# Sindhu-Hegde/jegal

Hardware: AMD Instinct MI355X
Metric: clips/sec (T=150 frames, 270x480) embedding extraction (higher is better)
Workload: dtype f16; 1 GPU; BASELINE configs[1]: synthetic batch=32 gesture-only (GestSync conv + JEGAL gesture encoder), uint8 150x270x480x3 clips resident in HBM, seeded synthetic weights; clips_per_gpu=32, frames=150, precision_mode=5, chunk=32, conv1_zero_tile_skip=True, dual_stream=True, parallelism=clip-sharded x1, no data-path collective

## Files before the change

### jegal_amd/csrc/conv1.hip

```cpp
#include "common.h"

#ifdef JG_CLOCK_STAMPS
__device__ unsigned long long jg_clock_stamps_conv1[2 * 1024];
extern "C" int jg_clock_read_conv1(unsigned long long* out, int n) {
    return hipMemcpyFromSymbol(out, HIP_SYMBOL(jg_clock_stamps_conv1), sizeof(unsigned long long) * (n < 2048 ? n : 2048)) == hipSuccess ? 0 : 1;
}
#endif
#include <cstdio>
#include <cstdlib>
#include <cstring>

struct Conv1Args {
    const uint8_t* src;
    int nclip, T, pad, P;
    const f16* Wd;
    float scale;
    f16* out;
    f16* edge;
    f16* dump;
    int nstrips;
    float invP;
    int zskip;
    const unsigned* zmask;
    const f16* zconst;
    int fill_partial;
};

namespace {
constexpr int IH = 270, IW = 480;
constexpr int PH = 43, PW = 78;
constexpr int TROWS = 16;
constexpr int ROW_PITCH = 3744;
constexpr int TILE_BYTES = TROWS * ROW_PITCH;
__device__ __host__ constexpr int slot_off(int x) { return 32 * x + 16 * (x / 3); }
constexpr int ROW_TILES = 22, COL_TILES = 5;
constexpr int CONV_BYTES = 4 * 8 * 32 * 16;
constexpr int CARRY_BYTES = 8 * 32 * 16;
constexpr int OFF_CONV = 2 * TILE_BYTES;
constexpr int OFF_CARRY = OFF_CONV + 2 * CONV_BYTES;
constexpr int OFF_INIT = OFF_CARRY + 2 * CARRY_BYTES;
constexpr int OFF_LIVE = OFF_INIT + 32;
constexpr int OFF_SKIP = OFF_INIT + 256;
constexpr int MAX_WG_STRIPS = 640;
constexpr int LDS_BYTES = OFF_SKIP + 4 * MAX_WG_STRIPS;
constexpr int MAX_WGS = 1024;
constexpr int DUMP_HALVES_PER_WG = 256 * 8;
}

typedef uint32_t u32x3 __attribute__((ext_vector_type(3)));
struct C1Regs { u32x3 w[2][5]; };

__device__ __forceinline__ f16x8 max8(f16x8 a, f16x8 b) {
    return __builtin_elementwise_max(a, b);
}

__device__ __forceinline__ int conv1_s2_of_mask(unsigned sk) {
    const int L = __builtin_ctz(~sk);
    constexpr int C2_OH = (PH - 5) / 2 + 1;
    const int rs = L >= 2 ? L - 2 : 0;
    return rs < C2_OH ? rs : C2_OH - 1;
}

struct Strips {
    int s_lo, r_hi, GX;
    const unsigned* tab;
    bool use_skip;
    __device__ __forceinline__ bool any() const { return s_lo < r_hi && GX > 0; }
    __device__ __forceinline__ unsigned zero_bands(int k) const {
        return use_skip ? (unsigned)__builtin_amdgcn_readfirstlane((int)tab[k]) : 0u;
    }
};
__device__ __forceinline__ Strips conv1_strips(const Conv1Args& a, const char* smem) {
    const int G32 = (int)gridDim.x;
    const int xcd = blockIdx.x & 7, xidx = blockIdx.x >> 3;
    const int GX = (G32 + 7 - xcd) >> 3;
    const int per = (a.nstrips + 7) >> 3;
    const int r_lo = xcd * per, r_hi = (r_lo + per < a.nstrips) ? r_lo + per : a.nstrips;
    return Strips{r_lo + xidx, r_hi, GX, reinterpret_cast<const unsigned*>(smem + OFF_SKIP), a.zmask != nullptr};
}
__device__ __forceinline__ void strip_split(int strip, int& nf, int& j) {
    nf = (int)((unsigned)strip / 5u);
    j = strip - nf * 5;
}
__device__ __forceinline__ unsigned skip_of(unsigned z) { return z & ((z << 1) | 1u); }
struct Walk {
    int strip, rt;
    int k;
    unsigned skip;
    unsigned z;
    bool done;
};
template <class F>
__device__ __forceinline__ void walk_next(const Strips& S, Walk& q, F&& on_strip) {
    if (q.done) return;
    while (true) {
        if (++q.rt == ROW_TILES) {
            q.rt = 0;
            q.strip += S.GX;
            ++q.k;
            if (q.strip >= S.r_hi) { q.done = true; return; }
            q.z = S.zero_bands(q.k);
            q.skip = skip_of(q.z);
            on_strip(q.strip, q.skip);
        }
        if (!((q.skip >> q.rt) & 1u)) return;
    }
}
template <class F>
__device__ __forceinline__ Walk walk_first(const Strips& S, F&& on_strip) {
    Walk q = {S.s_lo, -1, 0, 0u, 0u, !S.any()};
    if (q.done) return q;
    q.z = S.zero_bands(0);
    q.skip = skip_of(q.z);
    on_strip(q.strip, q.skip);
    walk_next(S, q, on_strip);
    return q;
}

__device__ __forceinline__ bool tile_live(const char* smem, int t) {
    return __builtin_amdgcn_readfirstlane(*reinterpret_cast<const int*>(smem + OFF_LIVE + (t & 1) * 4)) != 0;
}
__device__ __forceinline__ bool tile_is_zero(const char* smem, int t) {
    const int4 fl = *reinterpret_cast<const int4*>(smem + OFF_INIT + (t & 1) * 16);
    return __builtin_amdgcn_readfirstlane(fl.x | fl.y | fl.z | fl.w) == 0;
}

struct Mfma32 {
    static constexpr int NSTEP = 49, NCB = 1;
    static constexpr int DEPTH = 6;
    typedef f32x16 Acc;
    const int chalf, r, h;
    f16x8 wreg[49];
    const char* base;
    __device__ __forceinline__ Mfma32(const f16* Wd, int lane, int chalf_) : chalf(chalf_), r(lane & 31), h(lane >> 5) {
#pragma unroll
        for (int s = 0; s < 49; ++s)
            wreg[s] = *reinterpret_cast<const f16x8*>(Wd + conv1_wd_index(s, chalf * 32 + r, 8 * h));
    }
    __device__ __forceinline__ void set_tile(const char* cur) { base = cur + 112 * r + 16 * h; }
    __device__ __forceinline__ f16x8 frag(int gi) const {
        const int q = gi / 49, s = gi - q * 49;
        const int kh = s / 7, kw = s - kh * 7;
        return *reinterpret_cast<const f16x8*>(base + (6 * q + kh) * ROW_PITCH + 32 * kw + 16 * (kw / 3));
    }
    __device__ __forceinline__ static void zero(Acc& acc) {
#pragma unroll
        for (int x = 0; x < 16; ++x) acc[x] = 0.f;
    }
    __device__ __forceinline__ void step(Acc& acc, int s, int, f16x8 f) const {
        acc = __builtin_amdgcn_mfma_f32_32x32x16_f16(wreg[s], f, acc, 0, 0, 0);
    }
    __device__ __forceinline__ void store(const Acc& acc, char* cbuf, int mb, float scale) const {
#pragma unroll
        for (int g = 0; g < 4; ++g) {
            const f16x4 hv = {(f16)fmaxf(acc[4 * g] * scale, 0.f), (f16)fmaxf(acc[4 * g + 1] * scale, 0.f),
                              (f16)fmaxf(acc[4 * g + 2] * scale, 0.f), (f16)fmaxf(acc[4 * g + 3] * scale, 0.f)};
            *reinterpret_cast<f16x4*>(cbuf + ((mb * 8 + chalf * 4 + g) * 32 + r) * 16 + 8 * h) = hv;
        }
    }
};
struct Mfma16 {
    static constexpr int NSTEP = 25, NCB = 2;
    static constexpr int DEPTH = 4;
    struct Acc { f32x4 v[2][2]; };
    const int chalf, n16, kq, sel, half, colp;
    f16x8 wreg[25][2];
    int lb_row, lb_32, lb_224;
    int st_off;
    const char *p_row, *p_32, *p_224;
    __device__ __forceinline__ static void step_slots(int t, int& kha, int& kwa, int& khb, int& kwb) {
        if (t < 21) { kha = 2 * (t / 7); kwa = t % 7; khb = kha + 1; kwb = kwa; }
        else if (t == 21) { kha = khb = 6; kwa = 1; kwb = 2; }
        else if (t == 22) { kha = khb = 6; kwa = 4; kwb = 5; }
        else if (t == 23) { kha = khb = 6; kwa = 0; kwb = 6; }
        else { kha = khb = 6; kwa = 3; kwb = 4; }
    }
    __device__ __forceinline__ Mfma16(const f16* Wd, int lane, int chalf_)
        : chalf(chalf_), n16(lane & 15), kq(lane >> 4), sel(kq & 1), half(kq >> 1),
          colp((n16 >= 4 && n16 < 12) ? 2 * (n16 - 4) : (n16 < 4 ? 2 * n16 + 1 : 2 * (n16 - 8) + 1)) {
#pragma unroll
        for (int t = 0; t < 25; ++t) {
            int kha, kwa, khb, kwb;
            step_slots(t, kha, kwa, khb, kwb);
            const int sl = sel ? khb * 7 + kwb : kha * 7 + kwa;
#pragma unroll
            for (int ob = 0; ob < 2; ++ob) {
                wreg[t][ob] = *reinterpret_cast<const f16x8*>(Wd + conv1_wd_index(sl, chalf * 32 + ob * 16 + n16, 8 * half));
                if (t == 24 && sel) wreg[t][ob] = f16x8{0, 0, 0, 0, 0, 0, 0, 0};
            }
        }
        const int lb = 112 * colp + 16 * half;
        lb_row = lb + sel * ROW_PITCH; lb_32 = lb + sel * 32; lb_224 = lb + sel * 224;
        st_off = ((chalf * 4 + (kq >> 1)) * 32 + colp) * 16 + 8 * (kq & 1);
    }
    __device__ __forceinline__ void set_tile(const char* cur) {
        p_row = cur + lb_row;
        p_32 = cur + lb_32;
        p_224 = cur + lb_224;
    }
    __device__ __forceinline__ f16x8 frag(int gi) const {
        const int q = gi / 50, st = (gi - q * 50) >> 1, cb = gi & 1;
        int kha, kwa, khb, kwb;
        step_slots(st, kha, kwa, khb, kwb);
        const int off = (6 * q + kha) * ROW_PITCH + 32 * kwa + 16 * (kwa / 3) + 1792 * cb;
        const char* pb = st < 21 ? p_row : (st == 23 ? p_224 : p_32);
        return *reinterpret_cast<const f16x8*>(pb + off);
    }
    __device__ __forceinline__ static void zero(Acc& acc) {
#pragma unroll
        for (int ob = 0; ob < 2; ++ob)
#pragma unroll
            for (int cb = 0; cb < 2; ++cb) acc.v[ob][cb] = f32x4{0.f, 0.f, 0.f, 0.f};
    }
    __device__ __forceinline__ void step(Acc& acc, int st, int cb, f16x8 f) const {
        acc.v[0][cb] = __builtin_amdgcn_mfma_f32_16x16x32_f16(wreg[st][0], f, acc.v[0][cb], 0, 0, 0);
        acc.v[1][cb] = __builtin_amdgcn_mfma_f32_16x16x32_f16(wreg[st][1], f, acc.v[1][cb], 0, 0, 0);
    }
    __device__ __forceinline__ void store(const Acc& acc, char* cbuf, int mb, float scale) const {
#pragma unroll
        for (int ob = 0; ob < 2; ++ob)
#pragma unroll
            for (int cb = 0; cb < 2; ++cb) {
                const f32x4 v = acc.v[ob][cb];
                const f16x4 hv = {(f16)fmaxf(v.x * scale, 0.f), (f16)fmaxf(v.y * scale, 0.f), (f16)fmaxf(v.z * scale, 0.f), (f16)fmaxf(v.w * scale, 0.f)};
                *reinterpret_cast<f16x4*>(cbuf + st_off + ((mb * 8 + ob * 2) * 32 + cb * 16) * 16) = hv;
            }
    }
};

template <class Form>
__device__ __forceinline__ void conv1_mfma_role(const f16* Wd, float scale, char* smem, int lane, int wave) {
    constexpr int NSTEP = Form::NSTEP, NCB = Form::NCB, DEPTH = Form::DEPTH, NFRAG = 2 * NSTEP * NCB;
    const int mb0 = (wave >> 1) & 1;
    Form F(Wd, lane, wave & 1);
#ifdef JG_CLOCK_STAMPS
    const unsigned long long ck0 = __builtin_amdgcn_s_memtime(), rt0 = __builtin_amdgcn_s_memrealtime();
#endif
    for (int t = 0;; ++t) {
        __syncthreads();
        if (!tile_live(smem, t)) break;
        F.set_tile(smem + (t & 1) * TILE_BYTES + 3 * mb0 * ROW_PITCH);
        char* cbuf = smem + OFF_CONV + (t & 1) * CONV_BYTES;
        if (tile_is_zero(smem, t)) {
#pragma unroll
            for (int q = 0; q < 2; ++q) {
                typename Form::Acc acc;
                Form::zero(acc);
#pragma unroll
                for (int st = 0; st < 2; ++st)
#pragma unroll
                    for (int cb = 0; cb < NCB; ++cb) F.step(acc, st, cb, F.frag((q * NSTEP + st) * NCB + cb));
                F.store(acc, cbuf, mb0 + 2 * q, scale);
            }
            continue;
        }
        f16x8 fr[DEPTH];
#pragma unroll
        for (int gi = 0; gi < DEPTH; ++gi) fr[gi] = F.frag(gi);
#pragma unroll
        for (int q = 0; q < 2; ++q) {
            typename Form::Acc acc;
            Form::zero(acc);
#pragma unroll
            for (int st = 0; st < NSTEP; ++st)
#pragma unroll
                for (int cb = 0; cb < NCB; ++cb) {
                    const int gi = (q * NSTEP + st) * NCB + cb;
                    F.step(acc, st, cb, fr[gi % DEPTH]);
                    if (gi + DEPTH < NFRAG) fr[gi % DEPTH] = F.frag(gi + DEPTH);
                    __builtin_amdgcn_sched_barrier(0);
                }
            F.store(acc, cbuf, mb0 + 2 * q, scale);
        }
    }
#ifdef JG_CLOCK_STAMPS
    if (wave == 0 && lane == 0 && blockIdx.x < 1024) {
        jg_clock_stamps_conv1[2 * blockIdx.x] = __builtin_amdgcn_s_memtime() - ck0;
        jg_clock_stamps_conv1[2 * blockIdx.x + 1] = __builtin_amdgcn_s_memrealtime() - rt0;
    }
#endif
}

template <bool M16>
__global__ __launch_bounds__(512, 2) void conv1_direct_kernel(Conv1Args a) {
    extern __shared__ __attribute__((aligned(16))) char smem[];
    const int tid = threadIdx.x, lane = tid & 63;
    const int wave = __builtin_amdgcn_readfirstlane(tid >> 6);
    const Strips S = conv1_strips(a, smem);
    if (!S.any()) return;
    if (S.use_skip) {
        unsigned* tab = reinterpret_cast<unsigned*>(smem + OFF_SKIP);
        for (int k = tid; k < MAX_WG_STRIPS; k += 512) {
            const int strip = S.s_lo + k * S.GX;
            int nf, j;
            strip_split(strip, nf, j);
            tab[k] = strip < S.r_hi ? a.zmask[nf] : 0u;
        }
        __syncthreads();
    }
    if (wave >= 4) {
        const int ltid = tid - 256;
        const int row0 = ltid / 25, g0 = ltid - row0 * 25;
        const int it1 = ltid + 256;
        const bool has1 = it1 < TROWS * 25;
        const int row1 = has1 ? it1 / 25 : 0, g1 = has1 ? it1 - row1 * 25 : 0;

        uint32_t fb0_lo = (uint32_t)(uintptr_t)a.src, fb0_hi = (uint32_t)((uintptr_t)a.src >> 32);
        uint32_t fdelta[5] = {0, 0, 0, 0, 0};
        uint32_t ioff[2] = {0, 0};
        auto decode = [&](int strip, int& nf, int& j, int& b, int& pp) {
            strip_split(strip, nf, j);
            b = (int)((float)nf * a.invP);
            pp = nf - b * a.P;
            if (pp < 0) { --b; pp += a.P; }
            else if (pp >= a.P) { ++b; pp -= a.P; }
        };
        auto strip_setup = [&](int strip) {
            int nf, j, b, p;
            decode(strip, nf, j, b, p);
            int f0 = p - a.pad;
            f0 = f0 < 0 ? 0 : (f0 > a.T - 1 ? a.T - 1 : f0);
            const uintptr_t fb = (uintptr_t)(a.src + (size_t)(b * a.T + f0) * (size_t)(IH * IW * 3));
            fb0_lo = __builtin_amdgcn_readfirstlane((uint32_t)fb);
            fb0_hi = __builtin_amdgcn_readfirstlane((uint32_t)(fb >> 32));
#pragma unroll
            for (int dt = 0; dt < 5; ++dt) {
                int f = p + dt - a.pad;
                f = f < 0 ? 0 : (f > a.T - 1 ? a.T - 1 : f);
                fdelta[dt] = __builtin_amdgcn_readfirstlane((uint32_t)(f - f0) * (uint32_t)(IH * IW * 3));
            }
#pragma unroll
            for (int u = 0; u < 2; ++u) {
                const int row = u ? row1 : row0, g = u ? g1 : g0;
                int px = j * 96 + 4 * g;
                px = px < IW ? px : IW - 4;
                ioff[u] = (uint32_t)((row * IW + px) * 3);
            }
        };
        auto issue = [&](int rt, C1Regs& R) {
            const uint32_t roff = (uint32_t)rt * (uint32_t)(12 * IW * 3);
            const uint32_t o0 = ioff[0] + roff, o1 = ioff[1] + roff;
#pragma unroll
            for (int dt = 0; dt < 5; ++dt) {
                const uint8_t* fbu = reinterpret_cast<const uint8_t*>(((uintptr_t)fb0_lo | ((uintptr_t)fb0_hi << 32)) + fdelta[dt]);
                asm volatile("s_nop 4\n\tglobal_load_dwordx3 %0, %1, %2" : "=v"(R.w[0][dt]) : "v"(o0), "s"(fbu) : "memory");
                asm volatile("global_load_dwordx3 %0, %1, %2" : "=v"(R.w[1][dt]) : "v"(o1), "s"(fbu) : "memory");
            }
        };
        auto wait_frames = [&](C1Regs& R, int level) {
            if (level == 2) asm volatile("s_waitcnt vmcnt(11)" ::: "memory");
            else if (level == 1) asm volatile("s_waitcnt vmcnt(10)" ::: "memory");
            else asm volatile("s_waitcnt vmcnt(0)" ::: "memory");
#pragma unroll
            for (int u = 0; u < 2; ++u)
#pragma unroll
                for (int dt = 0; dt < 5; ++dt) asm volatile("" : "+v"(R.w[u][dt]));
        };
        bool zero_image[2] = {false, false};
        int* flags = reinterpret_cast<int*>(smem + OFF_INIT);
        auto cvt_write = [&](const C1Regs& R, char* buf, int slot, bool known_zero) {
            bool any;
            if (S.use_skip) {
                any = !known_zero;
            } else {
                uint32_t nz = 0;
#pragma unroll
                for (int u = 0; u < 2; ++u)
#pragma unroll
                    for (int dt = 0; dt < 5; ++dt) nz |= R.w[u][dt][0] | R.w[u][dt][1] | R.w[u][dt][2];
                any = !a.zskip || __builtin_amdgcn_ballot_w64(nz != 0) != 0;
            }
            if (lane == 0) flags[slot * 4 + (wave - 4)] = any ? 1 : 0;
            if (!any && zero_image[slot]) return;
            zero_image[slot] = !any;
#pragma unroll
            for (int u = 0; u < 2; ++u) {
                if (u == 1 && !has1) break;
                const int row = u ? row1 : row0, g = u ? g1 : g0;
#pragma unroll
                for (int q = 0; q < 4; ++q) {
                    uint32_t d[8];
#pragma unroll
                    for (int m = 0; m < 8; ++m) {
                        const int k0 = 2 * m, k1 = 2 * m + 1;
                        const int b0 = 3 * q + k0 % 3;
                        const uint32_t lo = R.w[u][k0 / 3][b0 >> 2];
                        if (k1 < 15) {
                            const int b1 = 3 * q + k1 % 3;
                            const uint32_t hi = R.w[u][k1 / 3][b1 >> 2];
                            d[m] = __builtin_amdgcn_perm(hi, lo, 0x0c000c00u | ((4u + (uint32_t)(b1 & 3)) << 16) | (uint32_t)(b0 & 3));
                        } else {
                            d[m] = __builtin_amdgcn_perm(CONV1_BIAS_ONE_BITS >> 8, lo, 0x040c0c00u | (uint32_t)(b0 & 3));
                        }
                    }
                    const int x = 4 * g + q;
                    char* dst = buf + row * ROW_PITCH + slot_off(x);
                    *reinterpret_cast<uint4*>(dst) = uint4{d[0], d[1], d[2], d[3]};
                    *reinterpret_cast<uint4*>(dst + 16) = uint4{d[4], d[5], d[6], d[7]};
                }
            }
        };
        const int pcg = (ltid >> 4) & 7, ppw = ltid & 15;
        f16* const dump = a.dump + ((long)blockIdx.x * 256 + ltid) * 8;
        const f16x8 cz = S.use_skip ? *reinterpret_cast<const f16x8*>(a.zconst + pcg * 8) : f16x8{0, 0, 0, 0, 0, 0, 0, 0};
        const int prow = __builtin_amdgcn_readfirstlane(ltid >> 7);
        const int ccol = ltid & 31, ccg = ltid >> 5;
        const int pthr = (prow * PW + ppw) * 64 + pcg * 8;
        auto pool = [&](int strip, int rt, int t, bool fastz, bool carry_const) {
            int nf, j;
            strip_split(strip, nf, j);
            const char* cbuf = smem + OFF_CONV + (t & 1) * CONV_BYTES;
            const char* cin = smem + OFF_CARRY + ((rt & 1) ^ 1) * CARRY_BYTES;
            char* cout = smem + OFF_CARRY + (rt & 1) * CARRY_BYTES;
            auto at = [&](const char* base, int row, int cg, int col) {
                return *reinterpret_cast<const f16x8*>(base + ((row * 8 + cg) * 32 + col) * 16);
            };
            const int c0 = 2 * ppw, c1 = c0 + 1, c2 = c0 + 2 < 32 ? c0 + 2 : 31;
            f16x8 m, cnext;
            if (fastz) {
                m = at(cbuf, 0, pcg, 0);
                cnext = at(cbuf, 0, ccg, 0);
            } else {
                const f16x8 q2 = at(cbuf, 2, ccg, ccol), q3 = at(cbuf, 3, ccg, ccol);
                cnext = max8(q2, q3);
                if (prow == 0) {
                    const f16x8 a0 = carry_const ? cz : at(cin, 0, pcg, c0), a1 = carry_const ? cz : at(cin, 0, pcg, c1),
                                a2 = carry_const ? cz : at(cin, 0, pcg, c2);
                    const f16x8 b0 = at(cbuf, 0, pcg, c0), b1 = at(cbuf, 0, pcg, c1), b2 = at(cbuf, 0, pcg, c2);
                    m = max8(max8(max8(a0, a1), max8(a2, b0)), max8(b1, b2));
                } else {
                    const f16x8 a0 = at(cbuf, 0, pcg, c0), a1 = at(cbuf, 0, pcg, c1), a2 = at(cbuf, 0, pcg, c2);
                    const f16x8 b0 = at(cbuf, 1, pcg, c0), b1 = at(cbuf, 1, pcg, c1), b2 = at(cbuf, 1, pcg, c2);
                    const f16x8 d0 = at(cbuf, 2, pcg, c0), d1 = at(cbuf, 2, pcg, c1), d2 = at(cbuf, 2, pcg, c2);
                    m = max8(max8(max8(a0, a1), max8(a2, b0)), max8(max8(b1, b2), max8(max8(d0, d1), d2)));
                }
            }
            const int ph = 2 * rt - 1 + prow;
            const int pw = 16 * j + ppw;
            {
                const long ub = ((long)nf * PH + (2 * rt - 1)) * (PW * 64) + j * (16 * 64);
                f16* dst = (ph >= 0 && pw < PW) ? a.out + ub + pthr : dump;
                __builtin_nontemporal_store(m, reinterpret_cast<f16x8*>(dst));
            }
            if (ph >= 0 && j > 0 && ppw == 0) {
                f16x8 e;
                if (fastz) e = m;
                else if (prow == 0) e = max8(carry_const ? cz : at(cin, 0, pcg, 0), at(cbuf, 0, pcg, 0));
                else e = max8(max8(at(cbuf, 0, pcg, 0), at(cbuf, 1, pcg, 0)), at(cbuf, 2, pcg, 0));
                *reinterpret_cast<f16x8*>(a.edge + (((long)nf * PH + ph) * 4 + (j - 1)) * 64 + pcg * 8) = e;
            }
            *reinterpret_cast<f16x8*>(cout + (ccg * 32 + ccol) * 16) = cnext;
        };
        auto fill_skipped = [&](int strip, unsigned skip) {
            if (!skip) return;
            const int fill_lo = a.fill_partial ? 2 * conv1_s2_of_mask(skip) : 0;
            int nf, j;
            strip_split(strip, nf, j);
            const int pw = 16 * j + ppw;
            for (unsigned m = skip; m; m &= m - 1) {
                const int rt = __builtin_ctz(m);
                const int ph = 2 * rt - 1 + prow;
                if (ph >= fill_lo && pw < PW)
                    *reinterpret_cast<f16x8*>(a.out + (((long)nf * PH + ph) * PW + pw) * 64 + pcg * 8) = cz;
                if (ph >= fill_lo && j > 0 && ppw == 0)
                    *reinterpret_cast<f16x8*>(a.edge + (((long)nf * PH + ph) * 4 + (j - 1)) * 64 + pcg * 8) = cz;
            }
        };

        int* live = reinterpret_cast<int*>(smem + OFF_LIVE);
        C1Regs RA, RB;
        struct Hist { int strip, rt; unsigned skip; bool zero; bool done; };
        auto on_strip = [&](int strip, unsigned skip) {
            strip_setup(strip);
            fill_skipped(strip, skip);
        };
        Walk qi = walk_first(S, on_strip);
        auto hist = [](const Walk& q) { return Hist{q.strip, q.rt, q.skip, q.rt >= 0 && ((q.z >> q.rt) & 1u) != 0, q.done}; };
        const Hist none = {0, 0, 0u, false, true};
        Hist hA = none, hB = none, hC = none, hD = none;
        int last_rt = 0;
        auto issue_next = [&](C1Regs& R) {
            hD = hC; hC = hB; hB = hA;
            hA = hist(qi);
            if (!qi.done) last_rt = qi.rt;
            issue(last_rt, R);
            walk_next(S, qi, on_strip);
        };
        if (ltid == 0) { live[0] = qi.done ? 0 : 1; live[1] = 0; }
        const bool any_tile = !qi.done;
        issue_next(RA);
        if (any_tile) {
            wait_frames(RA, 0);
            cvt_write(RA, smem, 0, hA.zero);
        }
        issue_next(RB);
        issue_next(RA);
        bool z1 = false, z2 = false;
        auto pool_step = [&](int tprev) {
            const bool above_skipped = hD.rt > 0 && ((hD.skip >> (hD.rt - 1)) & 1u);
            const bool above_zero = hD.rt == 0 || above_skipped || z2;
            pool(hD.strip, hD.rt, tprev, z1 && above_zero, above_skipped);
        };
        int t = 0;
        while (!hC.done) {
            __syncthreads();
            const bool zc0 = tile_is_zero(smem, t);
            if (ltid == 0) live[(t + 1) & 1] = hB.done ? 0 : 1;
            wait_frames(RB, t >= 2 ? 2 : 1);
            if (!hB.done) cvt_write(RB, smem + ((t + 1) & 1) * TILE_BYTES, (t + 1) & 1, hB.zero);
            if (t > 0) pool_step(t - 1);
            issue_next(RB);
            z2 = z1; z1 = zc0;
            ++t;
            if (hC.done) break;
            __syncthreads();
            const bool zc1 = tile_is_zero(smem, t);
            if (ltid == 0) live[(t + 1) & 1] = hB.done ? 0 : 1;
            wait_frames(RA, t >= 2 ? 2 : 1);
            if (!hB.done) cvt_write(RA, smem + ((t + 1) & 1) * TILE_BYTES, (t + 1) & 1, hB.zero);
            pool_step(t - 1);
            issue_next(RA);
            z2 = z1; z1 = zc1;
            ++t;
        }
        asm volatile("s_waitcnt vmcnt(0)" ::: "memory");
        __syncthreads();
        if (t > 0) pool_step(t - 1);
        return;
    }

    if constexpr (M16) conv1_mfma_role<Mfma16>(a.Wd, a.scale, smem, lane, wave);
    else conv1_mfma_role<Mfma32>(a.Wd, a.scale, smem, lane, wave);
}

__global__ void conv1_edge_fix_kernel(f16* __restrict__ out, const f16* __restrict__ edge, long n) {
    const long idx = blockIdx.x * (long)blockDim.x + threadIdx.x;
    if (idx >= n) return;
    const int cg = idx & 7;
    const int j = (idx >> 3) & 3;
    const long rowi = idx >> 5;
    f16* o = out + (rowi * PW + 16 * j + 15) * 64 + cg * 8;
    const f16x8 e = *reinterpret_cast<const f16x8*>(edge + (rowi * 4 + j) * 64 + cg * 8);
    *reinterpret_cast<f16x8*>(o) = max8(*reinterpret_cast<const f16x8*>(o), e);
}

__device__ __forceinline__ f16 conv1_zero_patch_value(const f16* __restrict__ Wd, float scale, int c) {
    const float hi = (float)Wd[conv1_wd_index(0, c, CONV1_BIAS_LANE)], lo = (float)Wd[conv1_wd_index(1, c, CONV1_BIAS_LANE)];
    const float acc = hi * CONV1_BIAS_ONE + lo * CONV1_BIAS_ONE;
    return (f16)fmaxf(acc * scale, 0.f);
}
__global__ void conv1_zconst_kernel(const f16* __restrict__ Wd, float scale, f16* __restrict__ zconst) {
    if (threadIdx.x < 64) zconst[threadIdx.x] = conv1_zero_patch_value(Wd, scale, threadIdx.x);
}

__global__ __launch_bounds__(256) void conv1_zero_scan_kernel(const uint8_t* __restrict__ src, unsigned* __restrict__ zmask,
                                                              const f16* __restrict__ Wd, float scale, f16* __restrict__ zconst) {
    __shared__ int rowz[IH + 2];
    const int tid = threadIdx.x, lane = tid & 63, wave = tid >> 6;
    const uint8_t* fb = src + (size_t)blockIdx.x * (size_t)(IH * IW * 3);
    for (int r = tid; r < IH; r += 256) {
        const uint4 v = *reinterpret_cast<const uint4*>(fb + (size_t)r * (IW * 3) + ((r * 37) % 90) * 16);
        rowz[r] = (v.x | v.y | v.z | v.w) == 0 ? 1 : 0;
    }
    __syncthreads();
    for (int r = wave; r < IH; r += 4) {
        if (!rowz[r]) continue;
        const uint8_t* row = fb + (size_t)r * (IW * 3);
        typedef unsigned u32x4 __attribute__((ext_vector_type(4)));
        u32x4 v = __builtin_nontemporal_load(reinterpret_cast<const u32x4*>(row + lane * 16));
        unsigned nz = v.x | v.y | v.z | v.w;
        if (lane < 26) {
            v = __builtin_nontemporal_load(reinterpret_cast<const u32x4*>(row + 1024 + lane * 16));
            nz |= v.x | v.y | v.z | v.w;
        }
        if (__builtin_amdgcn_ballot_w64(nz != 0) != 0 && lane == 0) rowz[r] = 0;
    }
    __syncthreads();
    if (wave == 0) {
        bool z = lane < ROW_TILES;
        if (z) {
            for (int r = 12 * lane; r < 12 * lane + TROWS; ++r) z = z && (r >= IH || rowz[r]);
        }
        const unsigned long long m = __builtin_amdgcn_ballot_w64(z);
        if (lane == 0) zmask[blockIdx.x] = (unsigned)m & ((1u << ROW_TILES) - 1u);
    }
    if (blockIdx.x == 0 && tid < 64) zconst[tid] = conv1_zero_patch_value(Wd, scale, tid);
    if (blockIdx.x == 0 && tid == 64) reinterpret_cast<int*>(zconst)[CONV1_ROWSKIP_WORD] = 0x7fffffff;
}

__global__ void conv1_skip_mask_kernel(const unsigned* __restrict__ fz, int nclip, int T, int pad, int P, unsigned* __restrict__ skip,
                                       int* __restrict__ s2, int* __restrict__ rowskip_min) {
    const int nf = blockIdx.x * blockDim.x + threadIdx.x;
    int rs = 0x7fffffff;
    if (nf < nclip * P) {
        const int b = nf / P, p = nf - b * P;
        unsigned z = (1u << ROW_TILES) - 1u;
        for (int dt = 0; dt < 5; ++dt) {
            int f = p + dt - pad;
            f = f < 0 ? 0 : (f > T - 1 ? T - 1 : f);
            z &= fz[b * T + f];
        }
        const unsigned sk = skip_of(z);
        skip[nf] = z;
        rs = conv1_s2_of_mask(sk);
        s2[nf] = rs;
    }
#pragma unroll
    for (int d = 32; d >= 1; d >>= 1) {
        const int o = __shfl_xor(rs, d, 64);
        rs = o < rs ? o : rs;
    }
    if ((threadIdx.x & 63) == 0 && rs != 0x7fffffff) atomicMin(rowskip_min, rs);
}

size_t conv1_zmask_elems(int nclip, int T) { return conv1_scan_view(nullptr, nclip, T, CONV1_SCAN_MAX_PAD).words; }
const int* conv1_s2_counts(const unsigned* zscratch, int nclip, int T, int pad) {
    return conv1_scan_view(const_cast<unsigned*>(zscratch), nclip, T, pad).s2();
}

hipError_t launch_conv1_scan(const uint8_t* src, int nclip, int T, int pad, const f16* Wd, float scale, unsigned* zscratch, hipStream_t s) {
    if (nclip * T <= 0) return hipSuccess;
    const int P = T + 2 * pad - 4;
    const Conv1Scan z = conv1_scan_view(zscratch, nclip, T, pad);
    hipLaunchKernelGGL(conv1_zero_scan_kernel, dim3((unsigned)(nclip * T)), dim3(256), 0, s, src, z.frame_mask(), Wd, scale * 16777216.0f,
                       static_cast<f16*>(z.zconst()));
    hipLaunchKernelGGL(conv1_skip_mask_kernel, dim3((unsigned)((nclip * P + 255) / 256)), dim3(256), 0, s, z.frame_mask(), nclip, T, pad, P,
                       z.pos_mask(), z.s2(), z.rowskip_min());
    return hipGetLastError();
}

hipError_t launch_conv1_zconst(const f16* Wd, float scale, f16* zconst, hipStream_t s) {
    hipLaunchKernelGGL(conv1_zconst_kernel, dim3(1), dim3(64), 0, s, Wd, scale * 16777216.0f, zconst);
    return hipGetLastError();
}

hipError_t launch_conv1_direct(const uint8_t* src, int nclip, int T, int pad, const f16* Wd, float scale,
                               f16* out_pooled, f16* edge, const unsigned* zscratch, bool fill_all, const EngineOpts& o, hipStream_t s) {
    static bool attr_set[64] = {};
    if (o.device < 0 || o.device >= 64) return hipErrorInvalidDevice;
    const int num_cu = o.num_cu;
    if (!attr_set[o.device]) {
        const void* ks[2] = {reinterpret_cast<const void*>(conv1_direct_kernel<false>), reinterpret_cast<const void*>(conv1_direct_kernel<true>)};
        for (const void* kf : ks) {
            hipError_t e = hipFuncSetAttribute(kf, hipFuncAttributeMaxDynamicSharedMemorySize, LDS_BYTES);
            if (e != hipSuccess) return e;
        }
        attr_set[o.device] = true;
    }
    Conv1Args a;
    a.src = src; a.nclip = nclip; a.T = T; a.pad = pad; a.P = T + 2 * pad - 4;
    a.dump = edge + (size_t)nclip * (T + 2 * pad - 4) * PH * 4 * 64;
    a.Wd = Wd; a.scale = scale * 16777216.0f; a.out = out_pooled; a.edge = edge;
    if ((long)nclip * a.P >= (1L << 24)) return hipErrorInvalidValue;
    a.nstrips = nclip * a.P * COL_TILES;
    a.invP = 1.0f / (float)a.P;
    a.zskip = o.conv1_zero_skip ? 1 : 0;
    a.zmask = nullptr;
    a.zconst = nullptr;
    a.fill_partial = 0;
    if (num_cu > MAX_WGS) return hipErrorInvalidValue;
    if (a.zskip && zscratch && nclip * T > 0 && (a.nstrips + num_cu - 1) / num_cu + 8 <= MAX_WG_STRIPS) {
        const Conv1Scan z = conv1_scan_view(const_cast<unsigned*>(zscratch), nclip, T, pad);
        a.zmask = z.pos_mask();
        a.zconst = static_cast<const f16*>(z.zconst());
        if (!fill_all) a.fill_partial = 1;
    }
    if (a.nstrips <= 0) return hipSuccess;
    if (num_cu < 8 && a.nstrips > num_cu) return hipErrorInvalidValue;
    const unsigned grid = (unsigned)(a.nstrips < num_cu ? a.nstrips : num_cu);
    if (o.conv1_mfma16) hipLaunchKernelGGL((conv1_direct_kernel<true>), dim3(grid), dim3(512), LDS_BYTES, s, a);
    else hipLaunchKernelGGL((conv1_direct_kernel<false>), dim3(grid), dim3(512), LDS_BYTES, s, a);
    return hipGetLastError();
}

hipError_t launch_conv1_edge_fix(f16* out_pooled, const f16* edge, long positions, hipStream_t s) {
    const long n = positions * PH * 4 * 8;
    if (n <= 0) return hipSuccess;
    hipLaunchKernelGGL(conv1_edge_fix_kernel, dim3((unsigned)((n + 255) / 256)), dim3(256), 0, s, out_pooled, edge, n);
    return hipGetLastError();
}

size_t conv1_edge_elems(long positions) { return (size_t)positions * PH * 4 * 64 + (size_t)MAX_WGS * DUMP_HALVES_PER_WG; }
```

Measured before the change: 2589 clips/s.

## Skip conv1 MFMA work per half-tile using per-row nonzero masks

The loader waves now record a per-row nonzero bitmask for each tile instead of a single any-nonzero flag, using a DPP wave OR reduction. The MFMA waves use that mask to replace each of the two output blocks with a cheap bias-only computation when its input rows are all zero, or when it is the bottom half of the last row tile. Partially zero tiles no longer run the full 49-step convolution on their zero half. Risks are the extra reduction cost in the loader, code growth from four unrolled branch variants, and correctness depending on the row-to-block mapping being right.

```diff
diff --git a/jegal_amd/csrc/conv1.hip b/jegal_amd/csrc/conv1.hip
--- a/jegal_amd/csrc/conv1.hip
+++ b/jegal_amd/csrc/conv1.hip
@@ -40,6 +40,8 @@
 constexpr int OFF_CARRY = OFF_CONV + 2 * CONV_BYTES;
 constexpr int OFF_INIT = OFF_CARRY + 2 * CARRY_BYTES;
 constexpr int OFF_LIVE = OFF_INIT + 32;
+constexpr int LIVE_TILE = 1, LIVE_LAST = 2;
+constexpr int BAND_FULL = 0, BAND_ZERO = 1, BAND_EDGE = 2;
 constexpr int OFF_SKIP = OFF_INIT + 256;
 constexpr int MAX_WG_STRIPS = 640;
 constexpr int LDS_BYTES = OFF_SKIP + 4 * MAX_WG_STRIPS;
@@ -117,12 +119,24 @@
     return q;
 }
 
-__device__ __forceinline__ bool tile_live(const char* smem, int t) {
-    return __builtin_amdgcn_readfirstlane(*reinterpret_cast<const int*>(smem + OFF_LIVE + (t & 1) * 4)) != 0;
+__device__ __forceinline__ int tile_live(const char* smem, int t) {
+    return __builtin_amdgcn_readfirstlane(*reinterpret_cast<const int*>(smem + OFF_LIVE + (t & 1) * 4));
 }
 __device__ __forceinline__ bool tile_is_zero(const char* smem, int t) {
     const int4 fl = *reinterpret_cast<const int4*>(smem + OFF_INIT + (t & 1) * 16);
     return __builtin_amdgcn_readfirstlane(fl.x | fl.y | fl.z | fl.w) == 0;
+}
+__device__ __forceinline__ unsigned tile_nonzero_rows(const char* smem, int t) {
+    const int4 fl = *reinterpret_cast<const int4*>(smem + OFF_INIT + (t & 1) * 16);
+    return (unsigned)__builtin_amdgcn_readfirstlane(fl.x | fl.y | fl.z | fl.w);
+}
+__device__ __forceinline__ unsigned wave_or(unsigned v) {
+    v |= (unsigned)__builtin_amdgcn_update_dpp(0, (int)v, 0xB1, 0xf, 0xf, true);
+    v |= (unsigned)__builtin_amdgcn_update_dpp(0, (int)v, 0x4E, 0xf, 0xf, true);
+    v |= (unsigned)__builtin_amdgcn_update_dpp(0, (int)v, 0x141, 0xf, 0xf, true);
+    v |= (unsigned)__builtin_amdgcn_update_dpp(0, (int)v, 0x140, 0xf, 0xf, true);
+    return (unsigned)(__builtin_amdgcn_readlane((int)v, 0) | __builtin_amdgcn_readlane((int)v, 16) | __builtin_amdgcn_readlane((int)v, 32) |
+                      __builtin_amdgcn_readlane((int)v, 48));
 }
 
 struct Mfma32 {
@@ -229,8 +243,42 @@
 };
 
 template <class Form>
-__device__ __forceinline__ void conv1_mfma_role(const f16* Wd, float scale, char* smem, int lane, int wave) {
-    constexpr int NSTEP = Form::NSTEP, NCB = Form::NCB, DEPTH = Form::DEPTH, NFRAG = 2 * NSTEP * NCB;
+__device__ __forceinline__ void conv1_bias_block(const Form& F, int q, char* cbuf, int mb, float scale) {
+    __builtin_amdgcn_sched_barrier(0);
+    typename Form::Acc acc;
+    Form::zero(acc);
+#pragma unroll
+    for (int st = 0; st < 2; ++st)
+#pragma unroll
+        for (int cb = 0; cb < Form::NCB; ++cb) F.step(acc, st, cb, F.frag((q * Form::NSTEP + st) * Form::NCB + cb));
+    F.store(acc, cbuf, mb, scale);
+    __builtin_amdgcn_sched_barrier(0);
+}
+template <class Form, int Q0, int NQ>
+__device__ __forceinline__ void conv1_live_blocks(const Form& F, char* cbuf, int mb0, float scale) {
+    constexpr int NSTEP = Form::NSTEP, NCB = Form::NCB, DEPTH = Form::DEPTH;
+    constexpr int G0 = Q0 * NSTEP * NCB, G1 = (Q0 + NQ) * NSTEP * NCB;
+    f16x8 fr[DEPTH];
+#pragma unroll
+    for (int gi = G0; gi < G0 + DEPTH; ++gi) fr[gi % DEPTH] = F.frag(gi);
+#pragma unroll
+    for (int q = Q0; q < Q0 + NQ; ++q) {
+        typename Form::Acc acc;
+        Form::zero(acc);
+#pragma unroll
+        for (int st = 0; st < NSTEP; ++st)
+#pragma unroll
+            for (int cb = 0; cb < NCB; ++cb) {
+                const int gi = (q * NSTEP + st) * NCB + cb;
+                F.step(acc, st, cb, fr[gi % DEPTH]);
+                if (gi + DEPTH < G1) fr[gi % DEPTH] = F.frag(gi + DEPTH);
+                __builtin_amdgcn_sched_barrier(0);
+            }
+        F.store(acc, cbuf, mb0 + 2 * q, scale);
+    }
+}
+template <class Form>
+__device__ __forceinline__ void conv1_mfma_role(const f16* Wd, float scale, int zskip, char* smem, int lane, int wave) {
     const int mb0 = (wave >> 1) & 1;
     Form F(Wd, lane, wave & 1);
 #ifdef JG_CLOCK_STAMPS
@@ -238,39 +286,28 @@
 #endif
     for (int t = 0;; ++t) {
         __syncthreads();
-        if (!tile_live(smem, t)) break;
+        const int lv = tile_live(smem, t);
+        if (!lv) break;
         F.set_tile(smem + (t & 1) * TILE_BYTES + 3 * mb0 * ROW_PITCH);
         char* cbuf = smem + OFF_CONV + (t & 1) * CONV_BYTES;
-        if (tile_is_zero(smem, t)) {
-#pragma unroll
-            for (int q = 0; q < 2; ++q) {
-                typename Form::Acc acc;
-                Form::zero(acc);
-#pragma unroll
-                for (int st = 0; st < 2; ++st)
-#pragma unroll
-                    for (int cb = 0; cb < NCB; ++cb) F.step(acc, st, cb, F.frag((q * NSTEP + st) * NCB + cb));
-                F.store(acc, cbuf, mb0 + 2 * q, scale);
-            }
-            continue;
-        }
-        f16x8 fr[DEPTH];
-#pragma unroll
-        for (int gi = 0; gi < DEPTH; ++gi) fr[gi] = F.frag(gi);
-#pragma unroll
-        for (int q = 0; q < 2; ++q) {
-            typename Form::Acc acc;
-            Form::zero(acc);
-#pragma unroll
-            for (int st = 0; st < NSTEP; ++st)
-#pragma unroll
-                for (int cb = 0; cb < NCB; ++cb) {
-                    const int gi = (q * NSTEP + st) * NCB + cb;
-                    F.step(acc, st, cb, fr[gi % DEPTH]);
-                    if (gi + DEPTH < NFRAG) fr[gi % DEPTH] = F.frag(gi + DEPTH);
-                    __builtin_amdgcn_sched_barrier(0);
-                }
-            F.store(acc, cbuf, mb0 + 2 * q, scale);
+        const unsigned rows = tile_nonzero_rows(smem, t) >> (3 * mb0);
+        const bool dead0 = (rows & 0x7fu) == 0;
+        const bool dead1 = ((rows >> 6) & 0x7fu) == 0 || (zskip && mb0 == 1 && (lv & LIVE_LAST));
+        if (dead0 && dead1) {
+            asm volatile("; conv1 blocks: dead dead" ::: "memory");
+            conv1_bias_block(F, 0, cbuf, mb0, scale);
+            conv1_bias_block(F, 1, cbuf, mb0 + 2, scale);
+        } else if (dead0) {
+            asm volatile("; conv1 blocks: dead live" ::: "memory");
+            conv1_bias_block(F, 0, cbuf, mb0, scale);
+            conv1_live_blocks<Form, 1, 1>(F, cbuf, mb0, scale);
+        } else if (dead1) {
+            asm volatile("; conv1 blocks: live dead" ::: "memory");
+            conv1_live_blocks<Form, 0, 1>(F, cbuf, mb0, scale);
+            conv1_bias_block(F, 1, cbuf, mb0 + 2, scale);
+        } else {
+            asm volatile("; conv1 blocks: live live" ::: "memory");
+            conv1_live_blocks<Form, 0, 2>(F, cbuf, mb0, scale);
         }
     }
 #ifdef JG_CLOCK_STAMPS
@@ -358,19 +395,23 @@
         };
         bool zero_image[2] = {false, false};
         int* flags = reinterpret_cast<int*>(smem + OFF_INIT);
-        auto cvt_write = [&](const C1Regs& R, char* buf, int slot, bool known_zero) {
-            bool any;
-            if (S.use_skip) {
-                any = !known_zero;
+        const unsigned rowbit0 = 1u << row0, rowbit1 = has1 ? 1u << row1 : 0u;
+        auto cvt_write = [&](const C1Regs& R, char* buf, int slot, int band) {
+            unsigned rows;
+            if (!a.zskip) {
+                rows = 0xffffu;
+            } else if (S.use_skip && band != BAND_EDGE) {
+                rows = band == BAND_ZERO ? 0u : 0xffffu;
             } else {
-                uint32_t nz = 0;
+                uint32_t nz[2] = {0, 0};
 #pragma unroll
                 for (int u = 0; u < 2; ++u)
 #pragma unroll
-                    for (int dt = 0; dt < 5; ++dt) nz |= R.w[u][dt][0] | R.w[u][dt][1] | R.w[u][dt][2];
-                any = !a.zskip || __builtin_amdgcn_ballot_w64(nz != 0) != 0;
-            }
-            if (lane == 0) flags[slot * 4 + (wave - 4)] = any ? 1 : 0;
+                    for (int dt = 0; dt < 5; ++dt) nz[u] |= R.w[u][dt][0] | R.w[u][dt][1] | R.w[u][dt][2];
+                rows = wave_or((nz[0] ? rowbit0 : 0u) | (nz[1] ? rowbit1 : 0u));
+            }
+            const bool any = rows != 0;
+            if (lane == 0) flags[slot * 4 + (wave - 4)] = (int)rows;
             if (!any && zero_image[slot]) return;
             zero_image[slot] = !any;
 #pragma unroll
@@ -468,15 +509,20 @@
         };
 
         int* live = reinterpret_cast<int*>(smem + OFF_LIVE);
+        auto live_word = [](int rt) { return LIVE_TILE | (rt == ROW_TILES - 1 ? LIVE_LAST : 0); };
         C1Regs RA, RB;
-        struct Hist { int strip, rt; unsigned skip; bool zero; bool done; };
+        struct Hist { int strip, rt; unsigned skip; int band; bool done; };
         auto on_strip = [&](int strip, unsigned skip) {
             strip_setup(strip);
             fill_skipped(strip, skip);
         };
         Walk qi = walk_first(S, on_strip);
-        auto hist = [](const Walk& q) { return Hist{q.strip, q.rt, q.skip, q.rt >= 0 && ((q.z >> q.rt) & 1u) != 0, q.done}; };
-        const Hist none = {0, 0, 0u, false, true};
+        auto hist = [](const Walk& q) {
+            const unsigned rt = (unsigned)(q.rt < 0 ? 0 : q.rt);
+            const int band = ((q.z >> rt) & 1u) ? BAND_ZERO : ((((q.z >> 1) | (q.z << 1)) >> rt) & 1u) ? BAND_EDGE : BAND_FULL;
+            return Hist{q.strip, q.rt, q.skip, band, q.done};
+        };
+        const Hist none = {0, 0, 0u, BAND_FULL, true};
         Hist hA = none, hB = none, hC = none, hD = none;
         int last_rt = 0;
         auto issue_next = [&](C1Regs& R) {
@@ -486,12 +532,12 @@
             issue(last_rt, R);
             walk_next(S, qi, on_strip);
         };
-        if (ltid == 0) { live[0] = qi.done ? 0 : 1; live[1] = 0; }
+        if (ltid == 0) { live[0] = qi.done ? 0 : live_word(qi.rt); live[1] = 0; }
         const bool any_tile = !qi.done;
         issue_next(RA);
         if (any_tile) {
             wait_frames(RA, 0);
-            cvt_write(RA, smem, 0, hA.zero);
+            cvt_write(RA, smem, 0, hA.band);
         }
         issue_next(RB);
         issue_next(RA);
@@ -505,9 +551,9 @@
         while (!hC.done) {
             __syncthreads();
             const bool zc0 = tile_is_zero(smem, t);
-            if (ltid == 0) live[(t + 1) & 1] = hB.done ? 0 : 1;
+            if (ltid == 0) live[(t + 1) & 1] = hB.done ? 0 : live_word(hB.rt);
             wait_frames(RB, t >= 2 ? 2 : 1);
-            if (!hB.done) cvt_write(RB, smem + ((t + 1) & 1) * TILE_BYTES, (t + 1) & 1, hB.zero);
+            if (!hB.done) cvt_write(RB, smem + ((t + 1) & 1) * TILE_BYTES, (t + 1) & 1, hB.band);
             if (t > 0) pool_step(t - 1);
             issue_next(RB);
             z2 = z1; z1 = zc0;
@@ -515,9 +561,9 @@
             if (hC.done) break;
             __syncthreads();
             const bool zc1 = tile_is_zero(smem, t);
-            if (ltid == 0) live[(t + 1) & 1] = hB.done ? 0 : 1;
+            if (ltid == 0) live[(t + 1) & 1] = hB.done ? 0 : live_word(hB.rt);
             wait_frames(RA, t >= 2 ? 2 : 1);
-            if (!hB.done) cvt_write(RA, smem + ((t + 1) & 1) * TILE_BYTES, (t + 1) & 1, hB.zero);
+            if (!hB.done) cvt_write(RA, smem + ((t + 1) & 1) * TILE_BYTES, (t + 1) & 1, hB.band);
             pool_step(t - 1);
             issue_next(RA);
             z2 = z1; z1 = zc1;
@@ -529,8 +575,8 @@
         return;
     }
 
-    if constexpr (M16) conv1_mfma_role<Mfma16>(a.Wd, a.scale, smem, lane, wave);
-    else conv1_mfma_role<Mfma32>(a.Wd, a.scale, smem, lane, wave);
+    if constexpr (M16) conv1_mfma_role<Mfma16>(a.Wd, a.scale, a.zskip, smem, lane, wave);
+    else conv1_mfma_role<Mfma32>(a.Wd, a.scale, a.zskip, smem, lane, wave);
 }
 
 __global__ void conv1_edge_fix_kernel(f16* __restrict__ out, const f16* __restrict__ edge, long n) {
```

After: 2568 clips/s, median of 2. About the same (-0.8%).
